# celliern/triflow

Hardware: AMD Instinct MI355X
Metric: implicit time-steps/s, 1e6-node 3-var system (member-steps/s over all GPUs) (higher is better)
Workload: dtype f64; 1 GPU; BASELINE config 3: M3_film, N=1000000 nodes, periodic, fixed dt=0.001, ROS2; members_per_gpu=1, parallelism=ensemble members sharded by rank, no data-path collective

## Files before the change

__graft_entry__.py:

```python
import os
import sys

ROOT = os.path.dirname(os.path.abspath(__file__))
if ROOT not in sys.path:
    sys.path.insert(0, ROOT)

PREBUILT = ["M1_advdiff", "M2_diff", "M3_film", "M5_stiff"]
PREBUILT_DENSE = ["M3_film", "M5_stiff"]
PREBUILT_CR_NARROW = ["M3_film", "M5_stiff", "tri3", "wide4"]


def build():
    from triflow_amd import compilers, workloads
    from triflow_amd.model import Model
    compilers.build_runtime_library()
    for name in PREBUILT:
        model = Model(*workloads.model_args(name), hold_compilation=True)
        for seg in (4, 8):
            compilers.build_code_object(model, 0, seg=seg)
    saved = os.environ.get("TRIFLOW_BLOCK_MASK")
    os.environ["TRIFLOW_BLOCK_MASK"] = "0"
    try:
        for name in PREBUILT_DENSE:
            model = Model(*workloads.model_args(name), hold_compilation=True)
            compilers.build_code_object(model, 0, seg=4)
    finally:
        if saved is None:
            del os.environ["TRIFLOW_BLOCK_MASK"]
        else:
            os.environ["TRIFLOW_BLOCK_MASK"] = saved
    from oracle import corpus
    for name in PREBUILT_CR_NARROW:
        model = Model(*corpus.model_args(name), hold_compilation=True)
        if name not in PREBUILT:
            compilers.build_code_object(model, 0, seg=4)
        with compilers.extra_flags("-DTF_CR_WIDE_IO=0"):
            compilers.build_code_object(model, 0, seg=4)
    import triflow_amd


def smoke():
    import numpy as np
    from triflow_amd import Model, schemes, workloads
    from oracle import numpy_path as ora
    name, fd, pars, dt, _ = workloads.config_inputs(3, 4096)
    model = Model(*workloads.model_args(name))
    ref = Model(*workloads.model_args(name), compiler=ora.numpy_compiler)
    F = model.F(model.fields_template(**fd), pars)
    Fo = ref.F(ref.fields_template(**fd), pars)
    assert np.array_equal(F, Fo), "F differs from the oracle"
    J = model.J(model.fields_template(**fd), pars)
    Jo = ref.J(ref.fields_template(**fd), pars)
    assert abs(J - Jo).max() <= 4 * np.spacing(abs(Jo).max()), "J differs from the oracle"
# ... 10 lines not shown
```

triflow_amd/codegen.py:

```python

import ast
import hashlib
import inspect
import os

import numpy as np
from sympy import lambdify

_FUNCS_1 = {"sqrt": "sqrt", "exp": "exp", "log": "log", "sin": "sin", "cos": "cos",
            "tan": "tan", "tanh": "tanh", "sinh": "sinh", "cosh": "cosh",
            "arctan": "atan", "arcsin": "asin", "arccos": "acos",
            "abs": "tf_abs", "absolute": "tf_abs", "fabs": "tf_abs", "sign": "tf_sign",
            "log10": "log10", "log2": "log2", "cbrt": "cbrt", "expm1": "expm1",
            "log1p": "log1p", "floor": "floor", "ceil": "ceil"}


class UnsupportedExpression(NotImplementedError):
    pass


HEAVISIDE_MODES = ("one", "exact")

_EXACT_HINT = '; Model(..., heaviside="exact") lowers Heaviside, DiracDelta and Piecewise exactly'

# ... 243 lines not shown
        names[name] = _c_ident(name)
        decls.append("const double %s = par[%d];" % (_c_ident(name), k))
    names["dx"] = "dx"
    names["x"] = "xc"
    uniform = {"dx"} | {name for k, name in enumerate(pars) if not (parvec_mask >> k) & 1}
    return names, decls, uniform


def block_mask(nvar, pat_eq, pat_var):
    if os.environ.get("TRIFLOW_BLOCK_MASK", "1") == "0":
        return [[True] * nvar for _ in range(nvar)]
    m = [[r == c for c in range(nvar)] for r in range(nvar)]
    for e, v in zip(pat_eq, pat_var):
        m[e][v] = True
    for k in range(nvar):
        for r in range(nvar):
            if m[r][k]:
                for c in range(nvar):
                    if m[k][c]:
                        m[r][c] = True
    return m


def lower_model(model, parvec_mask=0, seg=8, sweep_block=64):
    nvar = model._nvar
    fields = list(model._dep_vars) + list(model._help_funcs)
    nh = len(model._help_funcs)
    pars = list(model._pars)
    lo, hi = model._bounds
    mp = (model._window_range - 1) // 2
    if -lo != hi or hi != mp:
        raise UnsupportedExpression("asymmetric stencil window %r" % (model._bounds,))
    if mp < 1:
        mp = 1
    if nvar + nh > 16 or len(pars) > 16:
        raise UnsupportedExpression("too many fields / parameters for the HIP skeleton")
    if mp * nvar > 16:
        raise UnsupportedExpression(
            "the banded solver of the HIP back end handles b = (stencil half width) x (number of dependent "
            "variables) <= 16; this model has b = %d x %d = %d" % (mp, nvar, mp * nvar))
    sparse = [int(k) for k in model._sparse_indices[0]]
    nnz = len(sparse)
    real_mp = (model._window_range - 1) // 2
    pat_eq = [k % nvar for k in sparse]
    pat_var = [(k // nvar) % nvar for k in sparse]
    pat_off = [(k // nvar) // nvar - real_mp for k in sparse]
# ... 18 lines not shown
    uses_x = any("xc" in _tokens(s) for s in f_c + j_c + list(emit_f.denominators) + list(emit_j.denominators))

    j_uniform = [1 if emit_j.is_uniform(n) else 0 for n in j_nodes]

    j_alias, j_alias_scale = _proportional_entries(model, j_uniform, mode)

    def body(outname, exprs, emitter, only=None):
        lines = ["    " + d for d in decls if only is None or d.split("=")[1].strip().startswith("par[")]
        lines += ["    const double* tf_hc = par + %d;" % len(pars)]
        lines += ["    (void)dx; (void)xc; (void)par; (void)tf_hc;"]
        for den, k in sorted(emitter.denominators.items(), key=lambda kv: kv[1]) if only is None else ():
            lines += ["    const double tf_den%d = %s;" % (k, den),
                      "    const double tf_rden%d = 1.0 / tf_den%d;" % (k, k)]
        lines += ["    %s[%d] = %s;" % (outname, i, e) for i, e in enumerate(exprs)
                  if only is None or only[i]]
        return "\n".join(lines)

    def arr(name, values, ctype="int"):
        vals = ", ".join(str(v) for v in values) if values else "0"
        return "static constexpr %s %s[%d] = {%s};" % (ctype, name, max(len(values), 1), vals)

    blk_nz = block_mask(nvar, pat_eq, pat_var)
    blk_full = all(all(row) for row in blk_nz)
    hc_list = [src_ for src_, _ in sorted(host_consts.items(), key=lambda kv: kv[1])]
    par_is_vec = [1 if (parvec_mask >> k) & 1 else 0 for k in range(len(pars))] + [0] * len(hc_list)
    if len(pars) + len(hc_list) > 16:
        raise UnsupportedExpression("too many parameters + host constants for the HIP skeleton")
    src = "\n".join([
        "// generated by triflow_amd.codegen -- do not edit",
        "// equations: " + " ; ".join(str(e) for e in model._diff_eqs),
        *(["// heaviside: exact (Heaviside = numpy.heaviside, DiracDelta = 0, Piecewise = numpy.select)"]
          if mode == "exact" else []),
        "#define TF_NVAR %d" % nvar,
        "#define TF_NH %d" % nh,
        "#define TF_MP %d" % mp,
        "#define TF_NNZ %d" % nnz,
        "#define TF_NPAR %d" % (len(pars) + len(host_consts)),
        "#define TF_SEG %d" % seg,
        "#define TF_SWEEP_BLOCK %d" % sweep_block,
        "#define TF_USES_X %d" % (1 if uses_x else 0),
        arr("tf_pat_eq", pat_eq), arr("tf_pat_var", pat_var), arr("tf_pat_off", pat_off),
        "// entries of a solver block that can be non-zero (block_mask): [equation][variable]",
        "#define TF_BLK_FULL %d" % (1 if blk_full else 0),
        "static constexpr bool tf_blk_nz[%d][%d] = {%s};" % (
            nvar, nvar, ", ".join("{%s}" % ", ".join("true" if v else "false" for v in row) for row in blk_nz)),
        arr("tf_par_is_vec", par_is_vec, "bool"),
        arr("tf_j_uniform", j_uniform, "bool"),
        arr("tf_j_alias", j_alias), arr("tf_j_alias_scale", [_dbl(v) for v in j_alias_scale], "double"),
        "TF_DEVICE void tf_eval_F(const double (&w)[TF_NVAR + TF_NH][2 * TF_MP + 1], "
        "const double* par, double dx, double xc, double* F) {",
        body("F", f_c, emit_f),
        "}",
        "TF_DEVICE void tf_eval_J(const double (&w)[TF_NVAR + TF_NH][2 * TF_MP + 1], "
        "const double* par, double dx, double xc, double* J) {",
        body("J", j_c, emit_j),
        "}",
        "// the node-independent entries only (tf_j_uniform); same expressions, same bits",
        "TF_DEVICE void tf_eval_J_uniform(const double* par, double dx, double* J) {",
        "    const double xc = 0.0;",
        body("J", j_c, emit_j, only=j_uniform),
        "}",
        ""])
    spec = dict(nvar=nvar, nh=nh, npar=len(pars) + len(hc_list), npar_model=len(pars),
                host_consts=hc_list, mp=mp, nnz=nnz, seg=seg,
                sweep_block=sweep_block, uses_x=int(uses_x), parvec_mask=int(parvec_mask),
                b2=mp * nvar, pat_eq=pat_eq, pat_var=pat_var, pat_off=pat_off, j_uniform=j_uniform,
                j_alias=j_alias, j_alias_scale=j_alias_scale,
                blk_nz=blk_nz, fields=fields, pars=pars, heaviside=mode)
    return src, spec


PROBE_REDUCTIONS = ("sum", "mean", "integral", "max", "min", "argmax", "argmin")


def _lower_node_expressions(model, exprs, parvec_mask):
    fields = list(model._dep_vars) + list(model._help_funcs)
    pars = list(model._pars)
    mp = max((model._window_range - 1) // 2, 1)
    names, decls, uniform = _stencil_names(fields, pars, mp, parvec_mask)
    import sympy
    mode = heaviside_mode(model)
    for e in exprs:
        if mode == "one" and sympy.sympify(e).has(sympy.Heaviside):
            raise UnsupportedExpression("function 'Heaviside' is not supported in a probe or recorder: the HIP "
                                        "compiler takes it as identically one, as the reference does in J; "
                                        "write the step with Max / Min / sign" + _EXACT_HINT)
    nodes = _printed_expressions(model._symbolic_args, list(exprs), mode)
    first = _CEmitter(names, uniform, mode)
    for n in nodes:
        first.visit(n)
    emit = _CEmitter(names, uniform, mode)
# ... 215 lines not shown
```

triflow_amd/csrc/tf_kernels.h:

```cpp
#pragma once
#include "tf_args.h"

#ifndef TF_DEVICE
#error "define TF_DEVICE (e.g. __device__ __forceinline__) before including tf_kernels.h"
#endif

#define TF_W (2 * TF_MP + 1)
#define TF_NF (TF_NVAR + TF_NH)
#define TF_B2 (TF_MP * TF_NVAR)

#include "tf_math.h"

#if defined(TF_STAMPS) && defined(__HIP_DEVICE_COMPILE__)
#define TF_STAMP(a, i) do { if ((a).stamps && blockIdx.x == gridDim.x / 2 && threadIdx.x == 0) \
        (a).stamps[i] = __builtin_amdgcn_s_memtime(); } while (0)
#define TF_STAMP_T(a, i, tid) do { if ((a).stamps && blockIdx.x == gridDim.x / 2 && blockIdx.y == 0 && threadIdx.x == (tid)) \
        (a).stamps[i] = __builtin_amdgcn_s_memtime(); } while (0)
#define TF_STAMP_REAL(a, i) do { if ((a).stamps && blockIdx.x == gridDim.x / 2 && threadIdx.x == 0) \
        (a).stamps[i] = __builtin_amdgcn_s_memrealtime(); } while (0)
#define TF_STAMP_IF(a, i, cond) do { if ((a).stamps && (cond) && threadIdx.x == 0) (a).stamps[i] = __builtin_amdgcn_s_memtime(); } while (0)
#define TF_STAMP_REAL_IF(a, i, cond) do { if ((a).stamps && (cond) && threadIdx.x == 0) (a).stamps[i] = __builtin_amdgcn_s_memrealtime(); } while (0)
#define TF_COUNT(a, i) do { if ((a).stamps && (threadIdx.x & 63) == 0) atomicAdd(&(a).stamps[i], 1ull); } while (0)
#define TF_STAMP_L1(a, dir, i) do { if ((dir) > 0 && blockIdx.y == 0) TF_STAMP(a, i); } while (0)
#define TF_WGTRACE(a, k, which) do { if ((a).stamps && threadIdx.x == 0 && blockIdx.y * gridDim.x + blockIdx.x < 1024) \
        (a).stamps[512 + 2048 * (k) + 2 * (blockIdx.y * gridDim.x + blockIdx.x) + (which)] = __builtin_amdgcn_s_memrealtime(); } while (0)
#else
#define TF_STAMP_L1(a, dir, i) do {} while (0)
#define TF_WGTRACE(a, k, which) do {} while (0)
#define TF_STAMP(a, i) do {} while (0)
#define TF_STAMP_T(a, i, tid) do {} while (0)
#define TF_STAMP_REAL(a, i) do {} while (0)
#define TF_STAMP_IF(a, i, cond) do {} while (0)
// ... 487 lines not shown
#if defined(TF_BLK_FULL) && !TF_BLK_FULL
template <> struct TfMask<TF_NVAR> {
    static constexpr bool FULL = false;
    TF_DEVICE_M static constexpr bool nz(int r, int c) { return tf_blk_nz[r][c]; }
    TF_DEVICE_M static constexpr bool same(int r, int c) { return tf_blk_nz[r][c] && tf_blk_nz[c][r]; }
};
#endif

template <int B>
TF_DEVICE void tf_mm_sub(double (&C)[B][B], const double (&A)[B][B], const double (&Bm)[B][B]) {
    typedef TfMask<B> M;
#pragma unroll
    for (int r = 0; r < B; ++r)
#pragma unroll
        for (int c = 0; c < B; ++c) {
            if (!M::nz(r, c)) { C[r][c] = 0.0; continue; }
            double acc = C[r][c];
#pragma unroll
            for (int k = 0; k < B; ++k)
                if (M::nz(r, k) && M::nz(k, c)) acc = tf_fma(-A[r][k], Bm[k][c], acc);
            C[r][c] = acc;
        }
}
template <int B>
TF_DEVICE void tf_mm(double (&C)[B][B], const double (&A)[B][B], const double (&Bm)[B][B]) {
    typedef TfMask<B> M;
#pragma unroll
    for (int r = 0; r < B; ++r)
#pragma unroll
        for (int c = 0; c < B; ++c) {
            double acc = 0.0;
#pragma unroll
            for (int k = 0; k < B; ++k)
                if (M::nz(r, c) && M::nz(r, k) && M::nz(k, c)) acc = tf_fma(A[r][k], Bm[k][c], acc);
            C[r][c] = acc;
        }
}
template <int B>
TF_DEVICE void tf_mv_sub(double (&y)[B], const double (&A)[B][B], const double (&x)[B]) {
    typedef TfMask<B> M;
#pragma unroll
    for (int r = 0; r < B; ++r) {
        double acc = y[r];
#pragma unroll
        for (int k = 0; k < B; ++k)
            if (M::nz(r, k)) acc = tf_fma(-A[r][k], x[k], acc);
        y[r] = acc;
    }
}
template <int B>
TF_DEVICE void tf_mv(double (&y)[B], const double (&A)[B][B], const double (&x)[B]) {
    typedef TfMask<B> M;
#pragma unroll
    for (int r = 0; r < B; ++r) {
        double acc = 0.0;
#pragma unroll
        for (int k = 0; k < B; ++k)
// ... 115 lines not shown
                    if (d > gr) {
#pragma unroll
                        for (int t = TF_MP - 1; t >= 0; --t)
                            if (t == gr) {
#pragma unroll
                                for (int r = 0; r < TF_NVAR; ++r)
#pragma unroll
                                    for (int c = 0; c < TF_NVAR; ++c) {
                                        row[t + TF_MP][r][c] += row[d + TF_MP][r][c];
                                        row[d + TF_MP][r][c] = 0.0;
                                    }
                            }
                    }
            }
        }
#pragma unroll
        for (int r = 0; r < TF_NVAR; ++r) row[TF_MP][r][r] += 1.0;
    }
    TF_DEVICE_M void load(int i, double (&row)[2 * TF_MP + 1][TF_NVAR][TF_NVAR]) const {
        Raw raw;
        request(i, raw);
        decode(i, raw, row);
    }
};

template <int BB>
struct TfRowsBT {
    static constexpr int B = BB;
    static constexpr int MP = 1;
    static constexpr bool PIVOT = false;
    static constexpr bool MASKED = false;
    const TfLevelArgs& a;
    int pg, e, p, len, start;
    TF_DEVICE_M TfRowsBT(const TfLevelArgs& a_, int pg_) : a(a_), pg(pg_) {
        e = pg / a.L.P; p = pg - e * a.L.P;
        len = tf_len(a.L, p); start = tf_start(a.L, p);
    }
    struct Raw { double blk[3][BB][BB]; };
    TF_DEVICE_M void request(int i, Raw& r) const {
        const int64_t s = tf_idx(a.L, pg, i);
#pragma unroll
        for (int d = 0; d < 3; ++d)
#pragma unroll
            for (int rr = 0; rr < BB; ++rr)
#pragma unroll
                for (int c = 0; c < BB; ++c)
                    r.blk[d][rr][c] = a.Ablk[(int64_t)((d * BB + rr) * BB + c) * a.L.plane + s];
    }
    TF_DEVICE_M void decode(int i, const Raw& raw, double (&row)[3][BB][BB]) const {
#pragma unroll
        for (int d = 0; d < 3; ++d) tf_blk_copy<BB>(row[d], raw.blk[d]);
        if (!a.L.periodic) {
            const int g = start + i;
            if (g == 0) tf_blk_zero<BB>(row[0]);
            if (g == a.L.N - 1) tf_blk_zero<BB>(row[2]);
        }
    }
    TF_DEVICE_M void load(int i, double (&row)[3][BB][BB]) const {
        Raw raw;
        request(i, raw);
        decode(i, raw, row);
    }
};

template <class Rows>
TF_DEVICE_M constexpr bool tf_kept(int r, int k) { return !Rows::MASKED || TfMask<Rows::B>::nz(r, k); }

#define TF_PIN_REQUESTS() asm volatile("" ::: "memory")
#ifndef TF_BACKSUB_DEPTH
#define TF_BACKSUB_DEPTH 3
#endif
constexpr int tf_ring_depth(int nd, int other = 40) {
    return TF_BACKSUB_DEPTH * nd + other <= 240 ? TF_BACKSUB_DEPTH
         : (2 * nd + other <= 240 && TF_BACKSUB_DEPTH >= 2 ? 2 : 1);
}

template <int B, int MP>
TF_DEVICE int tf_twist_h(int mI, int enabled) {
    return (enabled && MP * B <= 6 && mI >= 4 * MP) ? (mI + 1) / 2 : mI;
}

template <class Rows, int DIR, bool MATRIX, bool DO_V = true, bool DO_W = true, bool DO_G = true>
TF_DEVICE void tf_asm_side(const TfLevelArgs& a, const Rows& own, int pg,
                           const double (&yN)[Rows::MP][Rows::B],
                           const double (&VN)[MATRIX ? Rows::MP : 1][MATRIX ? Rows::MP : 1][Rows::B][Rows::B],
                           const double (&WN)[MATRIX ? Rows::MP : 1][MATRIX ? Rows::MP : 1][Rows::B][Rows::B],
                           double* stage, int* rec) {
    constexpr int B = Rows::B, MP = Rows::MP, W = 2 * MP + 1, BB = MP * B;
    constexpr int VBLK = DIR > 0 ? 0 : 1, WBLK = 1 - VBLK;
// ... 132 lines not shown
    for (int k = 0; k < MP; ++k) {
        const int kn = DIR > 0 ? k : MP - 1 - k;
        if (DO_Y) {
#pragma unroll
            for (int r = 0; r < B; ++r) put(Tip::y(kn, r), yb[k][r]);
        }
        if (SPIKE) {
#pragma unroll
            for (int t = 0; t < MP; ++t) {
                const int tn = DIR > 0 ? t : MP - 1 - t;
#pragma unroll
                for (int r = 0; r < B; ++r)
#pragma unroll
                    for (int c = 0; c < B; ++c) {
                        const double vb = Vb[SPIKE ? k : 0][SPIKE ? t : 0][r][c];
                        const double wb = Wb[SPIKE ? k : 0][SPIKE ? t : 0][r][c];
                        if (DO_V) put(DIR > 0 ? Tip::V(kn, tn, r, c) : Tip::W(kn, tn, r, c), vb);
                        if (DO_W) put(DIR > 0 ? Tip::W(kn, tn, r, c) : Tip::V(kn, tn, r, c), wb);
                    }
            }
        }
    }
}

template <class Rows, int DIR, bool SPIKE, bool STORE_U, bool STORE_Y, bool KNOWN = false, bool YLDS = false,
          int ROLE = 0>
TF_DEVICE void tfk_chunk_body(const TfLevelArgs& a, int pg, double* ylds = nullptr,
                              double* asm_stage = nullptr, int* asm_rec = nullptr, double* xch = nullptr) {
    constexpr int B = Rows::B, MP = Rows::MP, W = 2 * MP + 1;
    static_assert(!KNOWN || (!SPIKE && !STORE_U), "the re-elimination takes one right-hand side");
    static_assert(ROLE == 0 || (SPIKE && !STORE_Y && !Rows::PIVOT), "the split walk carries spike columns and exchanges no rows");
    constexpr bool ES = SPIKE && ROLE == 0;
    constexpr int NX = (1 + MP) * B * B;
    constexpr bool PIV = Rows::PIVOT;
    constexpr int UW = PIV ? 2 * MP : MP;
    static_assert(!PIV || B == 1, "row exchanges are written for scalar blocks");
    typedef TfTips<B, MP> Tip;
    const TfLayout& L = a.L;
    if (pg >= L.Ptot) return;
    constexpr int SB = KNOWN ? 0 : (SPIKE ? 10 : 20);
    TF_STAMP_L1(a, DIR, SB + 0);
    Rows rows(a, pg);
    const int len = rows.len;
    const int mI = len - MP;
    auto node = [&](int j) { return DIR > 0 ? j : mI - 1 - j; };

// ... 99 lines not shown
                        Es[0][ES ? t : 0][0][0] = sw ? v : u; Es[ES ? q : 0][ES ? t : 0][0][0] = sw ? u : v;
                    }
                }
            }
        }
        {
            double Dinv[B][B];
            ok = tf_blk_inverse<B>(R[0][0], Dinv) && ok;
#pragma unroll
            for (int c = 1; c <= UW; ++c) tf_mm<B>(Un[c - 1], Dinv, R[0][c]);
            tf_mv<B>(yn, Dinv, y[0]);
            if (ES) {
#pragma unroll
                for (int t = 0; t < MP; ++t) tf_mm<B>(En[t], Dinv, Es[0][ES ? t : 0]);
            }
            if (ROLE == 1) {
                double* slot = xch + (j & 1) * (NX * 64);
#pragma unroll
                for (int r = 0; r < B; ++r)
#pragma unroll
                    for (int k = 0; k < B; ++k)
                        if (tf_kept<Rows>(r, k)) slot[(r * B + k) * 64] = Dinv[r][k];
            }
        }
        if (!PIV) fetch(MP, j + MP);
        if (ROLE == 1) {
            double* slot = xch + (j & 1) * (NX * 64);
#pragma unroll
            for (int q = 1; q <= MP; ++q)
#pragma unroll
                for (int r = 0; r < B; ++r)
#pragma unroll
                    for (int k = 0; k < B; ++k)
                        if (tf_kept<Rows>(r, k)) slot[((q * B + r) * B + k) * 64] = R[q][0][r][k];
            TF_WG_BARRIER();
        }
#pragma unroll
        for (int q = 1; q <= MP; ++q) {
#pragma unroll
            for (int c = 1; c <= UW; ++c) tf_mm_sub<B>(R[q][c], R[q][0], Un[c - 1]);
            tf_mv_sub<B>(y[q], R[q][0], yn);
            if (ES) {
#pragma unroll
                for (int t = 0; t < MP; ++t) tf_mm_sub<B>(Es[ES ? q : 0][ES ? t : 0], R[q][0], En[ES ? t : 0]);
            }
        }
        const bool keep = KNOWN || !a.respike;
        const bool keep_u = a.respike ? (DIR > 0 ? j < hdn : j < mI - hdn) : DIR > 0;
        if (STORE_U || STORE_Y) {
            const unsigned off = tf_off8(L, pg, node(j));
            if (STORE_U && keep_u) {
#pragma unroll
                for (int c = 0; c < UW; ++c)
#pragma unroll
                    for (int r = 0; r < B; ++r)
#pragma unroll
                        for (int k = 0; k < B; ++k) {
                            if (!tf_kept<Rows>(r, k)) continue;
                            tf_stp(a.Ut, (c * B + r) * B + k, L.plane, off, Un[c][r][k]);
                            if (ES && keep && c < MP)
                                tf_stp(a.Et, (c * B + r) * B + k, L.plane, off, En[ES && c < MP ? c : 0][r][k]);
                        }
            }
            if (STORE_Y && keep) {
                if (KNOWN && YLDS) {
#pragma unroll
                    for (int r = 0; r < B; ++r) ylds[(j * B + r) * 64] = yn[r];
                } else {
#pragma unroll
                    for (int r = 0; r < B; ++r) tf_stp(a.yt, r, L.plane, off, yn[r]);
                }
            }
        }
        if (HIST >= 0) {
            constexpr int H = HIST >= 0 ? HIST : 0;
#pragma unroll
            for (int c = 0; c < UW; ++c) tf_blk_copy<B>(Uh[H][c], Un[c]);
#pragma unroll
            for (int r = 0; r < B; ++r) yh[H][r] = yn[r];
            if (ES) {
#pragma unroll
                for (int t = 0; t < MP; ++t) tf_blk_copy<B>(Eh[ES ? H : 0][ES ? t : 0], En[ES ? t : 0]);
// ... 96 lines not shown
        double Dinv[B][B], En[MP][B][B], yn[B];
#pragma unroll
        for (int r = 0; r < B; ++r)
#pragma unroll
            for (int k = 0; k < B; ++k) Dinv[r][k] = tf_kept<Rows>(r, k) ? slot[(r * B + k) * 64] : 0.0;
        tf_mv<B>(yn, Dinv, y[0]);
#pragma unroll
        for (int t = 0; t < MP; ++t) tf_mm<B>(En[t], Dinv, Es[0][t]);
#pragma unroll
        for (int r = 0; r < B; ++r) y[MP][r] = ypre[r];
        request(j + MP + 1);
        TF_PIN_REQUESTS();
#pragma unroll
        for (int q = 1; q <= MP; ++q) {
            double M[B][B];
#pragma unroll
            for (int r = 0; r < B; ++r)
#pragma unroll
                for (int k = 0; k < B; ++k) M[r][k] = tf_kept<Rows>(r, k) ? slot[((q * B + r) * B + k) * 64] : 0.0;
            tf_mv_sub<B>(y[q], M, yn);
#pragma unroll
            for (int t = 0; t < MP; ++t) tf_mm_sub<B>(Es[q][t], M, En[t]);
        }
        const bool keep_u = a.respike ? (DIR > 0 ? j < hdn : j < mI - hdn) : DIR > 0;
        if ((STORE_U || STORE_Y) && !a.respike) {
            const unsigned off = tf_off8(L, pg, node(j));
            if (STORE_U && keep_u) {
#pragma unroll
                for (int c = 0; c < MP; ++c)
#pragma unroll
                    for (int r = 0; r < B; ++r)
#pragma unroll
                        for (int k = 0; k < B; ++k)
                            if (tf_kept<Rows>(r, k)) tf_stp(a.Et, (c * B + r) * B + k, L.plane, off, En[c][r][k]);
            }
            if (STORE_Y) {
#pragma unroll
                for (int r = 0; r < B; ++r) tf_stp(a.yt, r, L.plane, off, yn[r]);
            }
        }
        if (HIST >= 0) {
            constexpr int H = HIST >= 0 ? HIST : 0;
#pragma unroll
            for (int t = 0; t < MP; ++t) tf_blk_copy<B>(Eh[H][t], En[t]);
#pragma unroll
            for (int r = 0; r < B; ++r) yh[H][r] = yn[r];
        }
// ... 263 lines not shown
#pragma unroll
        for (int r = 0; r < B; ++r) xn[t][r] = 0.0;
    {
        int p2, i2;
        tf_locate(a.Lnext, p, p2, i2);
        const int64_t s2 = tf_idx(a.Lnext, e * a.Lnext.P + p2, i2);
#pragma unroll
        for (int t = 0; t < MP; ++t)
#pragma unroll
            for (int r = 0; r < B; ++r) xn[t][r] = a.xnext[tf_next_x(a, e, p, s2, t * B + r, MP * B)];
        tf_locate(a.Lnext, pa, p2, i2);
        const int64_t s2a = tf_idx(a.Lnext, e * a.Lnext.P + p2, i2);
#pragma unroll
        for (int t = 0; t < MP; ++t)
#pragma unroll
            for (int r = 0; r < B; ++r) sa[t][r] = has_above ? a.xnext[tf_next_x(a, e, pa, s2a, t * B + r, MP * B)] : 0.0;
    }
#pragma unroll
    for (int t = 0; t < MP; ++t) {
        const int64_t s = tf_idx(L, pg, mI + t);
#pragma unroll
        for (int r = 0; r < B; ++r) a.x[(int64_t)r * L.plane + s] = xn[t][r];
    }
    struct Node { double y[B]; double U[UW][B][B]; double E[WITH_E ? MP : 1][B][B]; };
    auto load = [&](int j, Node& n) {
        const unsigned off = tf_off8(L, pg, j);
#pragma unroll
        for (int r = 0; r < B; ++r) n.y[r] = tf_ldp(a.yt, r, L.plane, off);
#pragma unroll
        for (int c = 0; c < UW; ++c)
#pragma unroll
            for (int r = 0; r < B; ++r)
#pragma unroll
                for (int k = 0; k < B; ++k) {
                    const bool kept = tf_kept<Rows>(r, k);
                    n.U[c][r][k] = kept ? tf_ldp(a.Ut, (c * B + r) * B + k, L.plane, off) : 0.0;
                    if (WITH_E && c < MP) n.E[WITH_E && c < MP ? c : 0][r][k] = kept ? tf_ldp(a.Et, (c * B + r) * B + k, L.plane, off) : 0.0;
                }
    };
    constexpr int D = tf_ring_depth(B + UW * B * B + (WITH_E ? MP * B * B : 0));
    Node ring[D];
#pragma unroll
    for (int d = 0; d < D; ++d)
        if (mI - 1 - d >= 0) load(mI - 1 - d, ring[d]);
    for (int j0 = mI - 1; j0 >= 0; j0 -= D) {
#pragma unroll
        for (int d = 0; d < D; ++d) {
            const int j = j0 - d;
            if (j < 0) break;
            const Node& cur = ring[d];
            const int64_t s = tf_idx(L, pg, j);
            double x[B];
#pragma unroll
            for (int r = 0; r < B; ++r) x[r] = cur.y[r];
#pragma unroll
            for (int c = 0; c < UW; ++c) tf_mv_sub<B>(x, cur.U[c], xn[c]);
            if (WITH_E) {
#pragma unroll
                for (int c = 0; c < MP; ++c) tf_mv_sub<B>(x, cur.E[WITH_E ? c : 0], sa[c]);
            }
#pragma unroll
            for (int c = UW - 1; c > 0; --c)
#pragma unroll
                for (int r = 0; r < B; ++r) xn[c][r] = xn[c - 1][r];
#pragma unroll
            for (int r = 0; r < B; ++r) { xn[0][r] = x[r]; a.x[(int64_t)r * L.plane + s] = x[r]; }
            if (j - D >= 0) load(j - D, ring[d]);
        }
    }
}

template <int n>
TF_DEVICE bool tf_dense_solve(double (&S)[n][n], double (&g)[n]) {
    bool ok = true;
#pragma unroll
    for (int k = 0; k < n; ++k) {
#pragma unroll
        for (int r = k + 1; r < n; ++r) {
            const bool sw = tf_abs(S[r][k]) > tf_abs(S[k][k]);
// ... 16 lines not shown
        }
    }
#pragma unroll
    for (int k = n - 2; k >= 0; --k)
#pragma unroll
        for (int c = k + 1; c < n; ++c) g[k] = tf_fma(-S[k][c], g[c], g[k]);
    return ok;
}

template <class Rows, bool YLDS = false>
TF_DEVICE void tfk_backsub_twist_body(const TfLevelArgs& a, int pg, int dir,
                                      const double* ylds_dn = nullptr, const double* ylds_up = nullptr) {
    constexpr int B = Rows::B, MP = Rows::MP, NB = MP * B;
    static_assert(!Rows::PIVOT, "the re-elimination form is for block sizes that do not exchange rows");
    const TfLayout& L = a.L;
    if (pg >= L.Ptot) return;
    const int e = pg / L.P, p = pg - e * L.P;
    const int len = tf_len(L, p), mI = len - MP;
    const int h = tf_twist_h<B, MP>(mI, a.twist), hu = mI - h;
    if (dir == 1 && hu == 0) return;
    double xn[MP][B];
    const int jstart = hu == 0 ? mI - 1 : (dir == 0 ? h - MP - 1 : hu - MP - 1);
    auto nat = [&](int j) { return dir == 0 ? j : mI - 1 - j; };
    auto ldU = [&](int node_nat, double (&U)[MP][B][B], double (&y)[B]) {
        const unsigned off = tf_off8(L, pg, node_nat);
        if (YLDS) {
            const double* src = node_nat < h ? ylds_dn + node_nat * B * 64 : ylds_up + (mI - 1 - node_nat) * B * 64;
#pragma unroll
            for (int r = 0; r < B; ++r) y[r] = src[r * 64];
        } else {
#pragma unroll
            for (int r = 0; r < B; ++r) y[r] = tf_ldp(a.yt, r, L.plane, off);
        }
#pragma unroll
        for (int c = 0; c < MP; ++c)
#pragma unroll
            for (int r = 0; r < B; ++r)
#pragma unroll
                for (int k = 0; k < B; ++k)
                    U[c][r][k] = tf_kept<Rows>(r, k) ? tf_ldp(a.Ut, (c * B + r) * B + k, L.plane, off) : 0.0;
    };
    struct Upd { double b[B], k[B]; };
    const bool upd = YLDS && a.upd_n > 0;
    auto upd_load = [&](int nd, Upd& u) {
        if (upd) {
            const unsigned off = tf_off8(L, pg, nd);
#pragma unroll
            for (int r = 0; r < B; ++r) {
                u.b[r] = tf_ldp(a.upd_base, r, L.plane, off);
                u.k[r] = a.upd_n > 1 ? tf_ldp(a.upd_k0, r, L.plane, off) : 0.0;
            }
        }
    };
    auto emit = [&](int nd, const double (&x)[B], const Upd& u) {
        const int64_t s = tf_idx(L, pg, nd);
        if (upd) {
#pragma unroll
            for (int r = 0; r < B; ++r) {
                double acc;
                if (a.upd_n > 1) { acc = a.upd_c0 * u.k[r]; acc = acc + a.upd_c1 * x[r]; }
                else acc = a.upd_c0 * x[r];
                a.upd_out[(int64_t)r * L.plane + s] = u.b[r] + acc;
            }
        } else {
#pragma unroll
            for (int r = 0; r < B; ++r) a.x[(int64_t)r * L.plane + s] = x[r];
        }
    };
    double xsep[MP][B], xmid[MP][B];
    const bool own_sep = hu == 0 || dir == 0;
    if (own_sep) {
        int p2, i2;
        tf_locate(a.Lnext, p, p2, i2);
        const int64_t s2 = tf_idx(a.Lnext, e * a.Lnext.P + p2, i2);
#pragma unroll
        for (int t = 0; t < MP; ++t) {
#pragma unroll
            for (int r = 0; r < B; ++r) {
                const double v = a.xnext[tf_next_x(a, e, p, s2, t * B + r, MP * B)];
                xn[t][r] = v;
                xsep[t][r] = v;
            }
        }
    }
    struct Node { double y[B]; double U[MP][B][B]; Upd u; };
    auto load = [&](int j, Node& n) { ldU(nat(j), n.U, n.y); upd_load(nat(j), n.u); };
    constexpr int D = tf_ring_depth(3 * B + MP * B * B, 2 * (MP * B) * (MP * B) + 2 * MP * B + MP * B * B + B);
    Node ring[D];
#pragma unroll
    for (int d = 0; d < D; ++d)
        if (jstart - d >= 0) load(jstart - d, ring[d]);
    if (hu != 0) {
        double Tc[NB][NB], Tg[NB];
        double S[NB][NB], g2[NB];
        double Uk[MP][B][B], yk[B];
#pragma unroll
        for (int k = MP - 1; k >= 0; --k) {
            ldU(h - MP + k, Uk, yk);
#pragma unroll
            for (int i = 0; i < B; ++i) {
                Tg[k * B + i] = yk[i];
#pragma unroll
                for (int c = 0; c < NB; ++c) { Tc[k * B + i][c] = 0.0; }
            }
#pragma unroll
            for (int c = 0; c < MP; ++c) {
                const int u = k + 1 + c;
                if (u >= MP) {
#pragma unroll
                    for (int i = 0; i < B; ++i)
#pragma unroll
                        for (int jj = 0; jj < B; ++jj) Tc[k * B + i][(u - MP) * B + jj] += Uk[c][i][jj];
                } else {
#pragma unroll
                    for (int i = 0; i < B; ++i)
#pragma unroll
                        for (int jj = 0; jj < B; ++jj) {
                            const double f = Uk[c][i][jj];
                            Tg[k * B + i] = tf_fma(-f, Tg[u * B + jj], Tg[k * B + i]);
#pragma unroll
                            for (int cc = 0; cc < NB; ++cc)
                                Tc[k * B + i][cc] = tf_fma(-f, Tc[u * B + jj][cc], Tc[k * B + i][cc]);
                        }
                }
            }
        }
#pragma unroll
        for (int k = 0; k < MP; ++k) {
            ldU(h + k, Uk, yk);
#pragma unroll
            for (int i = 0; i < B; ++i) {
                g2[k * B + i] = yk[i];
#pragma unroll
                for (int c = 0; c < NB; ++c) S[k * B + i][c] = (c == k * B + i) ? 1.0 : 0.0;
            }
#pragma unroll
            for (int c = 0; c < MP; ++c) {
                const int u = MP + k - 1 - c;
                if (u >= MP) {
#pragma unroll
                    for (int i = 0; i < B; ++i)
#pragma unroll
                        for (int jj = 0; jj < B; ++jj) S[k * B + i][(u - MP) * B + jj] += Uk[c][i][jj];
                } else if (u >= 0) {
#pragma unroll
                    for (int i = 0; i < B; ++i)
#pragma unroll
                        for (int jj = 0; jj < B; ++jj) {
                            const double f = Uk[c][i][jj];
                            g2[k * B + i] = tf_fma(-f, Tg[u * B + jj], g2[k * B + i]);
#pragma unroll
                            for (int cc = 0; cc < NB; ++cc)
// ... 17 lines not shown
        } else {
#pragma unroll
            for (int k = 0; k < MP; ++k)
#pragma unroll
                for (int r = 0; r < B; ++r) { xmid[k][r] = g2[k * B + r]; xn[MP - 1 - k][r] = g2[k * B + r]; }
        }
    }
    Upd usep[MP], umid[MP];
#pragma unroll
    for (int t = 0; t < MP; ++t) {
        if (own_sep) upd_load(mI + t, usep[t]);
        if (hu != 0) upd_load(dir == 0 ? h - MP + t : h + t, umid[t]);
    }
    for (int j0 = jstart; j0 >= 0; j0 -= D) {
#pragma unroll
        for (int d = 0; d < D; ++d) {
            const int j = j0 - d;
            if (j < 0) break;
            const Node& cur = ring[d];
            double x[B];
#pragma unroll
            for (int r = 0; r < B; ++r) x[r] = cur.y[r];
#pragma unroll
            for (int c = 0; c < MP; ++c) tf_mv_sub<B>(x, cur.U[c], xn[c]);
#pragma unroll
            for (int c = MP - 1; c > 0; --c)
#pragma unroll
                for (int r = 0; r < B; ++r) xn[c][r] = xn[c - 1][r];
#pragma unroll
            for (int r = 0; r < B; ++r) xn[0][r] = x[r];
            emit(nat(j), x, cur.u);
            if (j - D >= 0) load(j - D, ring[d]);
        }
    }
#pragma unroll
    for (int t = 0; t < MP; ++t) {
        if (own_sep) emit(mI + t, xsep[t], usep[t]);
        if (hu != 0) emit(dir == 0 ? h - MP + t : h + t, xmid[t], umid[t]);
    }
}

#define TF_TINY_MAXN (2 * TF_MP * TF_NVAR)
TF_DEVICE void tfk_tiny_factor_body(const TfTinyArgs& a, int e) {
    const TfLayout& L = a.L;
    if (e >= L.nsys) return;
    const int N = L.N, n = N * TF_NVAR;
    double* A = a.lu + (int64_t)e * n * n;
// ... 93 lines not shown
```

Before: 2702 steps/s.

## Store outermost U block in factored form, recompute from Dinv and Jacobian planes

Instead of storing the full outermost off-diagonal U block per node, the forward sweep stores only the Dinv columns that reach the outer offset. The back-substitution reloads those columns plus the Jacobian value planes feeding the outer block and rebuilds that block with a small masked matrix product. This cuts global-memory traffic for U in the memory-bound banded solve, at the cost of extra loads of Jacobian planes and a few extra FMAs per node. It also adds an environment switch and prebuilds variants with it disabled.

```diff
diff --git a/__graft_entry__.py b/__graft_entry__.py
--- a/__graft_entry__.py
+++ b/__graft_entry__.py
@@ -8,6 +8,21 @@
 PREBUILT = ["M1_advdiff", "M2_diff", "M3_film", "M5_stiff"]
 PREBUILT_DENSE = ["M3_film", "M5_stiff"]
 PREBUILT_CR_NARROW = ["M3_film", "M5_stiff", "tri3", "wide4"]
+PREBUILT_U_STORED = ["M3_film"]
+U_OUTER_SYNTH = (["-dxv", "u*dxxxu + k*dxxv"], ["u", "v"], ["k"], None)
+
+
+def _with_env(pairs, fn):
+    saved = {k: os.environ.get(k) for k in pairs}
+    os.environ.update(pairs)
+    try:
+        return fn()
+    finally:
+        for k, v in saved.items():
+            if v is None:
+                del os.environ[k]
+            else:
+                os.environ[k] = v
 
 
 def build():
@@ -18,17 +33,17 @@
         model = Model(*workloads.model_args(name), hold_compilation=True)
         for seg in (4, 8):
             compilers.build_code_object(model, 0, seg=seg)
-    saved = os.environ.get("TRIFLOW_BLOCK_MASK")
-    os.environ["TRIFLOW_BLOCK_MASK"] = "0"
-    try:
-        for name in PREBUILT_DENSE:
+    for name in PREBUILT_DENSE:
+        model = Model(*workloads.model_args(name), hold_compilation=True)
+        _with_env(dict(TRIFLOW_BLOCK_MASK="0"), lambda: compilers.build_code_object(model, 0, seg=4))
+    for name in PREBUILT_U_STORED:
+        for mask in ("1", "0"):
             model = Model(*workloads.model_args(name), hold_compilation=True)
-            compilers.build_code_object(model, 0, seg=4)
-    finally:
-        if saved is None:
-            del os.environ["TRIFLOW_BLOCK_MASK"]
-        else:
-            os.environ["TRIFLOW_BLOCK_MASK"] = saved
+            _with_env(dict(TRIFLOW_U_OUTER="0", TRIFLOW_BLOCK_MASK=mask),
+                      lambda: compilers.build_code_object(model, 0, seg=4))
+    for u_outer in ("1", "0"):
+        model = Model(*U_OUTER_SYNTH, hold_compilation=True)
+        _with_env(dict(TRIFLOW_U_OUTER=u_outer), lambda: compilers.build_code_object(model, 0, seg=4))
     from oracle import corpus
     for name in PREBUILT_CR_NARROW:
         model = Model(*corpus.model_args(name), hold_compilation=True)
diff --git a/triflow_amd/codegen.py b/triflow_amd/codegen.py
--- a/triflow_amd/codegen.py
+++ b/triflow_amd/codegen.py
@@ -289,6 +289,51 @@
     return m
 
 
+REGISTER_BLOCK_MAX = 6
+
+
+def outer_u_form(nvar, mp, pat_eq, pat_var, pat_off, j_uniform, j_alias, blk_nz):
+    if os.environ.get("TRIFLOW_U_OUTER", "1") == "0" or nvar < 2 or mp * nvar > REGISTER_BLOCK_MAX:
+        return None
+    nnz = len(pat_eq)
+    form = dict(nz=[], rows=[], planes=[])
+    for off in (mp, -mp):
+        ks = [k for k in range(nnz) if pat_off[k] == off]
+        nz = [[False] * nvar for _ in range(nvar)]
+        for k in ks:
+            nz[pat_eq[k]][pat_var[k]] = True
+        rows = [any(nz[e]) for e in range(nvar)]
+        planes = sorted({(j_alias[k] if j_alias[k] >= 0 else k) for k in ks if not j_uniform[k]})
+        stored = sum(1 for r in range(nvar) for k in range(nvar) if rows[k] and blk_nz[r][k])
+        block = sum(1 for r in range(nvar) for c in range(nvar) if blk_nz[r][c])
+        if not stored + len(planes) < block:
+            return None
+        form["nz"].append(nz)
+        form["rows"].append(rows)
+        form["planes"].append(planes)
+    return form
+
+
+def _outer_u_lines(form, nvar, nnz):
+    if form is None:
+        return []
+
+    def bools(values):
+        return "{%s}" % ", ".join("true" if v else "false" for v in values)
+    return [
+        "// outermost block of the stored pivot rows in factored form (outer_u_form); [0]: offset +mp, [1]: -mp",
+        "#define TF_UOUT_FACT 1",
+        "// pattern of the outer block of A: [direction][equation][variable]",
+        "static constexpr bool tf_uout_nz[2][%d][%d] = {%s};" % (
+            nvar, nvar, ", ".join("{%s}" % ", ".join(bools(row) for row in nz) for nz in form["nz"])),
+        "// S, the equations that reach the outer offset: the columns of Dinv that are stored",
+        "static constexpr bool tf_uout_row[2][%d] = {%s};" % (nvar, ", ".join(bools(r) for r in form["rows"])),
+        "// the value planes that feed the outer block",
+        "static constexpr bool tf_uout_ld[2][%d] = {%s};" % (
+            max(nnz, 1), ", ".join(bools([k in planes for k in range(max(nnz, 1))]) for planes in form["planes"])),
+    ]
+
+
 def lower_model(model, parvec_mask=0, seg=8, sweep_block=64):
     nvar = model._nvar
     fields = list(model._dep_vars) + list(model._help_funcs)
@@ -353,6 +398,7 @@
 
     blk_nz = block_mask(nvar, pat_eq, pat_var)
     blk_full = all(all(row) for row in blk_nz)
+    u_outer = outer_u_form(nvar, mp, pat_eq, pat_var, pat_off, j_uniform, j_alias, blk_nz)
     hc_list = [src_ for src_, _ in sorted(host_consts.items(), key=lambda kv: kv[1])]
     par_is_vec = [1 if (parvec_mask >> k) & 1 else 0 for k in range(len(pars))] + [0] * len(hc_list)
     if len(pars) + len(hc_list) > 16:
@@ -378,6 +424,7 @@
         arr("tf_par_is_vec", par_is_vec, "bool"),
         arr("tf_j_uniform", j_uniform, "bool"),
         arr("tf_j_alias", j_alias), arr("tf_j_alias_scale", [_dbl(v) for v in j_alias_scale], "double"),
+        *_outer_u_lines(u_outer, nvar, nnz),
         "TF_DEVICE void tf_eval_F(const double (&w)[TF_NVAR + TF_NH][2 * TF_MP + 1], "
         "const double* par, double dx, double xc, double* F) {",
         body("F", f_c, emit_f),
@@ -397,7 +444,7 @@
                 sweep_block=sweep_block, uses_x=int(uses_x), parvec_mask=int(parvec_mask),
                 b2=mp * nvar, pat_eq=pat_eq, pat_var=pat_var, pat_off=pat_off, j_uniform=j_uniform,
                 j_alias=j_alias, j_alias_scale=j_alias_scale,
-                blk_nz=blk_nz, fields=fields, pars=pars, heaviside=mode)
+                blk_nz=blk_nz, u_outer=u_outer, fields=fields, pars=pars, heaviside=mode)
     return src, spec
 
 
diff --git a/triflow_amd/csrc/tf_kernels.h b/triflow_amd/csrc/tf_kernels.h
--- a/triflow_amd/csrc/tf_kernels.h
+++ b/triflow_amd/csrc/tf_kernels.h
@@ -8,6 +8,9 @@
 #define TF_W (2 * TF_MP + 1)
 #define TF_NF (TF_NVAR + TF_NH)
 #define TF_B2 (TF_MP * TF_NVAR)
+#ifndef TF_UOUT_FACT
+#define TF_UOUT_FACT 0
+#endif
 
 #include "tf_math.h"
 
@@ -541,8 +544,9 @@
             C[r][c] = acc;
         }
 }
-template <int B>
-TF_DEVICE void tf_mm(double (&C)[B][B], const double (&A)[B][B], const double (&Bm)[B][B]) {
+struct TfEveryTerm { TF_DEVICE_M constexpr bool operator()(int) const { return true; } };
+template <int B, class Term = TfEveryTerm>
+TF_DEVICE void tf_mm(double (&C)[B][B], const double (&A)[B][B], const double (&Bm)[B][B], Term term = Term()) {
     typedef TfMask<B> M;
 #pragma unroll
     for (int r = 0; r < B; ++r)
@@ -551,7 +555,7 @@
             double acc = 0.0;
 #pragma unroll
             for (int k = 0; k < B; ++k)
-                if (M::nz(r, c) && M::nz(r, k) && M::nz(k, c)) acc = tf_fma(A[r][k], Bm[k][c], acc);
+                if (M::nz(r, c) && M::nz(r, k) && M::nz(k, c) && term(k)) acc = tf_fma(A[r][k], Bm[k][c], acc);
             C[r][c] = acc;
         }
 }
@@ -713,6 +717,33 @@
         request(i, raw);
         decode(i, raw, row);
     }
+#if TF_UOUT_FACT
+    TF_DEVICE_M void request_outer(int i, bool up, Raw& r) const {
+        const unsigned off = tf_off8(a.L, pg, i);
+#pragma unroll
+        for (int k = 0; k < TF_NNZ; ++k) {
+            if (TF_JU(k)) r.jv[k] = ju.v[k];
+            else if (tf_uout_ld[0][k] && tf_uout_ld[1][k]) r.jv[k] = tf_ldp(a.Jv, k, a.L.plane, off);
+            else if (tf_uout_ld[0][k] || tf_uout_ld[1][k]) {
+                if (up == tf_uout_ld[1][k]) r.jv[k] = tf_ldp(a.Jv, k, a.L.plane, off);
+            }
+        }
+    }
+    TF_DEVICE_M void decode_outer(int i, bool up, const Raw& raw, double (&blk)[TF_NVAR][TF_NVAR]) const {
+        tf_blk_zero<TF_NVAR>(blk);
+#pragma unroll
+        for (int k = 0; k < TF_NNZ; ++k) {
+            if (tf_pat_off[k] != TF_MP && tf_pat_off[k] != -TF_MP) continue;
+            if (up != (tf_pat_off[k] < 0)) continue;
+            const double jv = TF_JA(k) ? tf_j_alias_scale[k] * raw.jv[tf_j_alias[k] >= 0 ? tf_j_alias[k] : 0] : raw.jv[k];
+            blk[tf_pat_eq[k]][tf_pat_var[k]] = -a.c * jv;
+        }
+        if (!a.L.periodic) {
+            const int gl = start + i, gr = a.L.N - 1 - gl;
+            if (up ? gl < TF_MP : gr < TF_MP) tf_blk_zero<TF_NVAR>(blk);
+        }
+    }
+#endif
 };
 
 template <int BB>
@@ -756,6 +787,57 @@
 
 template <class Rows>
 TF_DEVICE_M constexpr bool tf_kept(int r, int k) { return !Rows::MASKED || TfMask<Rows::B>::nz(r, k); }
+
+template <class Rows> struct TfUOut {
+    static constexpr bool ON = false;
+    TF_DEVICE_M static constexpr bool row(bool, int) { return true; }
+    static constexpr int RING = Rows::B * Rows::B;
+};
+#if TF_UOUT_FACT
+constexpr int tf_uout_count(int dir) {
+    int n = 0;
+    for (int k = 0; k < TF_NVAR; ++k) n += tf_uout_row[dir][k] ? TF_NVAR : 0;
+    for (int k = 0; k < TF_NNZ; ++k) n += tf_uout_ld[dir][k] ? 1 : 0;
+    return n;
+}
+template <> struct TfUOut<TfRowsL1> {
+    static constexpr bool ON = true;
+    static_assert(!TfRowsL1::PIVOT, "exchanged rows do not keep their outermost block");
+    TF_DEVICE_M static constexpr bool row(bool up, int k) { return up ? tf_uout_row[1][k] : tf_uout_row[0][k]; }
+    static constexpr int RING = tf_uout_count(0) > tf_uout_count(1) ? tf_uout_count(0) : tf_uout_count(1);
+};
+#endif
+
+template <class Rows, int UW, bool FACT = TfUOut<Rows>::ON> struct TfULoad {
+    static constexpr bool FACTORED = false;
+    struct Outer {};
+    TF_DEVICE_M TfULoad(const TfLevelArgs&, int) {}
+};
+template <class Rows, int UW> struct TfULoad<Rows, UW, true> {
+    static constexpr int B = Rows::B;
+    static constexpr bool FACTORED = true;
+    typedef typename Rows::Raw Outer;
+    Rows rows;
+    TF_DEVICE_M TfULoad(const TfLevelArgs& a, int pg) : rows(a, pg) {}
+    TF_DEVICE_M void request(const TfLevelArgs& a, unsigned off, int i, bool up, double (&U)[UW][B][B], Outer& o) const {
+#pragma unroll
+        for (int c = 0; c < UW; ++c)
+#pragma unroll
+            for (int r = 0; r < B; ++r)
+#pragma unroll
+                for (int k = 0; k < B; ++k) {
+                    U[c][r][k] = 0.0;
+                    if (tf_kept<Rows>(r, k) && (c < UW - 1 || TfUOut<Rows>::row(up, k)))
+                        U[c][r][k] = tf_ldp(a.Ut, (c * B + r) * B + k, a.L.plane, off);
+                }
+        rows.request_outer(i, up, o);
+    }
+    TF_DEVICE_M void outer(int i, bool up, const double (&U)[UW][B][B], const Outer& o, double (&Uo)[B][B]) const {
+        double A[B][B];
+        rows.decode_outer(i, up, o, A);
+        tf_mm<B>(Uo, U[UW - 1], A, [up](int k) { return TfUOut<Rows>::row(up, k); });
+    }
+};
 
 #define TF_PIN_REQUESTS() asm volatile("" ::: "memory")
 #ifndef TF_BACKSUB_DEPTH
@@ -934,6 +1016,8 @@
         }
     }
 }
+
+#define TF_KEEP_U(a, DIR, j, hdn, mI) ((a).respike ? ((DIR) > 0 ? (j) < (hdn) : (j) < (mI) - (hdn)) : (DIR) > 0)
 
 template <class Rows, int DIR, bool SPIKE, bool STORE_U, bool STORE_Y, bool KNOWN = false, bool YLDS = false,
           int ROLE = 0>
@@ -1079,6 +1163,17 @@
                     for (int k = 0; k < B; ++k)
                         if (tf_kept<Rows>(r, k)) slot[(r * B + k) * 64] = Dinv[r][k];
             }
+            if constexpr (TfUOut<Rows>::ON && STORE_U) {
+                if (TF_KEEP_U(a, DIR, j, hdn, mI)) {
+                    const unsigned off = tf_off8(L, pg, node(j));
+#pragma unroll
+                    for (int r = 0; r < B; ++r)
+#pragma unroll
+                        for (int k = 0; k < B; ++k)
+                            if (tf_kept<Rows>(r, k) && TfUOut<Rows>::row(DIR < 0, k))
+                                tf_stp(a.Ut, ((UW - 1) * B + r) * B + k, L.plane, off, Dinv[r][k]);
+                }
+            }
         }
         if (!PIV) fetch(MP, j + MP);
         if (ROLE == 1) {
@@ -1103,7 +1198,7 @@
             }
         }
         const bool keep = KNOWN || !a.respike;
-        const bool keep_u = a.respike ? (DIR > 0 ? j < hdn : j < mI - hdn) : DIR > 0;
+        const bool keep_u = TF_KEEP_U(a, DIR, j, hdn, mI);
         if (STORE_U || STORE_Y) {
             const unsigned off = tf_off8(L, pg, node(j));
             if (STORE_U && keep_u) {
@@ -1114,7 +1209,8 @@
 #pragma unroll
                         for (int k = 0; k < B; ++k) {
                             if (!tf_kept<Rows>(r, k)) continue;
-                            tf_stp(a.Ut, (c * B + r) * B + k, L.plane, off, Un[c][r][k]);
+                            if (!TfUOut<Rows>::ON || c < UW - 1)
+                                tf_stp(a.Ut, (c * B + r) * B + k, L.plane, off, Un[c][r][k]);
                             if (ES && keep && c < MP)
                                 tf_stp(a.Et, (c * B + r) * B + k, L.plane, off, En[ES && c < MP ? c : 0][r][k]);
                         }
@@ -1257,7 +1353,7 @@
 #pragma unroll
             for (int t = 0; t < MP; ++t) tf_mm_sub<B>(Es[q][t], M, En[t]);
         }
-        const bool keep_u = a.respike ? (DIR > 0 ? j < hdn : j < mI - hdn) : DIR > 0;
+        const bool keep_u = TF_KEEP_U(a, DIR, j, hdn, mI);
         if ((STORE_U || STORE_Y) && !a.respike) {
             const unsigned off = tf_off8(L, pg, node(j));
             if (STORE_U && keep_u) {
@@ -1567,23 +1663,36 @@
 #pragma unroll
         for (int r = 0; r < B; ++r) a.x[(int64_t)r * L.plane + s] = xn[t][r];
     }
-    struct Node { double y[B]; double U[UW][B][B]; double E[WITH_E ? MP : 1][B][B]; };
+    typedef TfULoad<Rows, UW> ULoad;
+    const ULoad uload(a, pg);
+    struct Node : ULoad::Outer { double y[B]; double U[UW][B][B]; double E[WITH_E ? MP : 1][B][B]; };
     auto load = [&](int j, Node& n) {
         const unsigned off = tf_off8(L, pg, j);
 #pragma unroll
         for (int r = 0; r < B; ++r) n.y[r] = tf_ldp(a.yt, r, L.plane, off);
-#pragma unroll
-        for (int c = 0; c < UW; ++c)
-#pragma unroll
-            for (int r = 0; r < B; ++r)
-#pragma unroll
-                for (int k = 0; k < B; ++k) {
-                    const bool kept = tf_kept<Rows>(r, k);
-                    n.U[c][r][k] = kept ? tf_ldp(a.Ut, (c * B + r) * B + k, L.plane, off) : 0.0;
-                    if (WITH_E && c < MP) n.E[WITH_E && c < MP ? c : 0][r][k] = kept ? tf_ldp(a.Et, (c * B + r) * B + k, L.plane, off) : 0.0;
-                }
+        if constexpr (ULoad::FACTORED) {
+            uload.request(a, off, j, false, n.U, n);
+#pragma unroll
+            for (int c = 0; c < (WITH_E ? MP : 0); ++c)
+#pragma unroll
+                for (int r = 0; r < B; ++r)
+#pragma unroll
+                    for (int k = 0; k < B; ++k)
+                        n.E[c][r][k] = tf_kept<Rows>(r, k) ? tf_ldp(a.Et, (c * B + r) * B + k, L.plane, off) : 0.0;
+        } else {
+#pragma unroll
+            for (int c = 0; c < UW; ++c)
+#pragma unroll
+                for (int r = 0; r < B; ++r)
+#pragma unroll
+                    for (int k = 0; k < B; ++k) {
+                        const bool kept = tf_kept<Rows>(r, k);
+                        n.U[c][r][k] = kept ? tf_ldp(a.Ut, (c * B + r) * B + k, L.plane, off) : 0.0;
+                        if (WITH_E && c < MP) n.E[WITH_E && c < MP ? c : 0][r][k] = kept ? tf_ldp(a.Et, (c * B + r) * B + k, L.plane, off) : 0.0;
+                    }
+        }
     };
-    constexpr int D = tf_ring_depth(B + UW * B * B + (WITH_E ? MP * B * B : 0));
+    constexpr int D = tf_ring_depth(B + (UW - 1) * B * B + TfUOut<Rows>::RING + (WITH_E ? MP * B * B : 0));
     Node ring[D];
 #pragma unroll
     for (int d = 0; d < D; ++d)
@@ -1599,7 +1708,12 @@
 #pragma unroll
             for (int r = 0; r < B; ++r) x[r] = cur.y[r];
 #pragma unroll
-            for (int c = 0; c < UW; ++c) tf_mv_sub<B>(x, cur.U[c], xn[c]);
+            for (int c = 0; c < (ULoad::FACTORED ? UW - 1 : UW); ++c) tf_mv_sub<B>(x, cur.U[c], xn[c]);
+            if constexpr (ULoad::FACTORED) {
+                double Uo[B][B];
+                uload.outer(j, false, cur.U, cur, Uo);
+                tf_mv_sub<B>(x, Uo, xn[UW - 1]);
+            }
             if (WITH_E) {
 #pragma unroll
                 for (int c = 0; c < MP; ++c) tf_mv_sub<B>(x, cur.E[WITH_E ? c : 0], sa[c]);
@@ -1662,7 +1776,9 @@
     double xn[MP][B];
     const int jstart = hu == 0 ? mI - 1 : (dir == 0 ? h - MP - 1 : hu - MP - 1);
     auto nat = [&](int j) { return dir == 0 ? j : mI - 1 - j; };
-    auto ldU = [&](int node_nat, double (&U)[MP][B][B], double (&y)[B]) {
+    typedef TfULoad<Rows, MP> ULoad;
+    const ULoad uload(a, pg);
+    auto ldU = [&](int node_nat, double (&U)[MP][B][B], double (&y)[B], typename ULoad::Outer& o) {
         const unsigned off = tf_off8(L, pg, node_nat);
         if (YLDS) {
             const double* src = node_nat < h ? ylds_dn + node_nat * B * 64 : ylds_up + (mI - 1 - node_nat) * B * 64;
@@ -1672,13 +1788,26 @@
 #pragma unroll
             for (int r = 0; r < B; ++r) y[r] = tf_ldp(a.yt, r, L.plane, off);
         }
-#pragma unroll
-        for (int c = 0; c < MP; ++c)
-#pragma unroll
-            for (int r = 0; r < B; ++r)
-#pragma unroll
-                for (int k = 0; k < B; ++k)
-                    U[c][r][k] = tf_kept<Rows>(r, k) ? tf_ldp(a.Ut, (c * B + r) * B + k, L.plane, off) : 0.0;
+        if constexpr (ULoad::FACTORED) {
+            uload.request(a, off, node_nat, node_nat >= h, U, o);
+        } else {
+#pragma unroll
+            for (int c = 0; c < MP; ++c)
+#pragma unroll
+                for (int r = 0; r < B; ++r)
+#pragma unroll
+                    for (int k = 0; k < B; ++k)
+                        U[c][r][k] = tf_kept<Rows>(r, k) ? tf_ldp(a.Ut, (c * B + r) * B + k, L.plane, off) : 0.0;
+        }
+    };
+    auto ldU_whole = [&](int node_nat, double (&U)[MP][B][B], double (&y)[B]) {
+        typename ULoad::Outer o;
+        ldU(node_nat, U, y, o);
+        if constexpr (ULoad::FACTORED) {
+            double Uo[B][B];
+            uload.outer(node_nat, node_nat >= h, U, o, Uo);
+            tf_blk_copy<B>(U[MP - 1], Uo);
+        }
     };
     struct Upd { double b[B], k[B]; };
     const bool upd = YLDS && a.upd_n > 0;
@@ -1723,9 +1852,10 @@
             }
         }
     }
-    struct Node { double y[B]; double U[MP][B][B]; Upd u; };
-    auto load = [&](int j, Node& n) { ldU(nat(j), n.U, n.y); upd_load(nat(j), n.u); };
-    constexpr int D = tf_ring_depth(3 * B + MP * B * B, 2 * (MP * B) * (MP * B) + 2 * MP * B + MP * B * B + B);
+    struct Node : ULoad::Outer { double y[B]; double U[MP][B][B]; Upd u; };
+    auto load = [&](int j, Node& n) { ldU(nat(j), n.U, n.y, n); upd_load(nat(j), n.u); };
+    constexpr int D = tf_ring_depth(3 * B + (MP - 1) * B * B + TfUOut<Rows>::RING,
+                                    2 * (MP * B) * (MP * B) + 2 * MP * B + MP * B * B + B);
     Node ring[D];
 #pragma unroll
     for (int d = 0; d < D; ++d)
@@ -1736,7 +1866,7 @@
         double Uk[MP][B][B], yk[B];
 #pragma unroll
         for (int k = MP - 1; k >= 0; --k) {
-            ldU(h - MP + k, Uk, yk);
+            ldU_whole(h - MP + k, Uk, yk);
 #pragma unroll
             for (int i = 0; i < B; ++i) {
                 Tg[k * B + i] = yk[i];
@@ -1767,7 +1897,7 @@
         }
 #pragma unroll
         for (int k = 0; k < MP; ++k) {
-            ldU(h + k, Uk, yk);
+            ldU_whole(h + k, Uk, yk);
 #pragma unroll
             for (int i = 0; i < B; ++i) {
                 g2[k * B + i] = yk[i];
@@ -1831,7 +1961,12 @@
 #pragma unroll
             for (int r = 0; r < B; ++r) x[r] = cur.y[r];
 #pragma unroll
-            for (int c = 0; c < MP; ++c) tf_mv_sub<B>(x, cur.U[c], xn[c]);
+            for (int c = 0; c < (ULoad::FACTORED ? MP - 1 : MP); ++c) tf_mv_sub<B>(x, cur.U[c], xn[c]);
+            if constexpr (ULoad::FACTORED) {
+                double Uo[B][B];
+                uload.outer(nat(j), dir != 0, cur.U, cur, Uo);
+                tf_mv_sub<B>(x, Uo, xn[MP - 1]);
+            }
 #pragma unroll
             for (int c = MP - 1; c > 0; --c)
 #pragma unroll
```

After: 2763 steps/s (median of 6 runs). 2.3% higher.
